# tlepoint/fhe.rs

Measured on NVIDIA B200. Metric: bfv_ct_mul_relin_per_sec_n32768_14x62bit, higher is better.
Workload: dtype u64

## Files before the change

### bench_micro/mac_bench.cu

```cuda
#include <cstdio>
#include <cuda_runtime.h>
typedef unsigned long long u64;
typedef unsigned int u32;

template <int V>
struct Acc {
  u32 e0, e1, e2, e3, e4, o1, o2, o3;
  u64 lo, mid, hi;
  __device__ __forceinline__ void clear() { e0 = e1 = e2 = e3 = e4 = o1 = o2 = o3 = 0; lo = mid = hi = 0; }
  __device__ __forceinline__ void mac(u64 a, u64 b) {
    if (V == 0) {
      asm volatile("{\n\t.reg .u32 a0,a1,b0,b1;\n\tmov.b64 {a0,a1}, %3;\n\tmov.b64 {b0,b1}, %4;\n\t"
          "mad.wide.u32 %0, a0, b0, %0;\n\tmad.wide.u32 %1, a0, b1, %1;\n\tmad.wide.u32 %1, a1, b0, %1;\n\tmad.wide.u32 %2, a1, b1, %2;\n\t}"
          : "+l"(lo), "+l"(mid), "+l"(hi) : "l"(a), "l"(b));
    } else if (V == 1) {
      asm volatile("{\n\t.reg .u32 a0, a1, b0, b1;\n\tmov.b64 {a0, a1}, %8;\n\tmov.b64 {b0, b1}, %9;\n\t"
          "mad.lo.cc.u32 %0, a0, b0, %0;\n\tmadc.hi.cc.u32 %1, a0, b0, %1;\n\tmadc.lo.cc.u32 %2, a1, b1, %2;\n\t"
          "madc.hi.cc.u32 %3, a1, b1, %3;\n\taddc.u32 %4, %4, 0;\n\t"
          "mad.lo.cc.u32 %5, a0, b1, %5;\n\tmadc.hi.cc.u32 %6, a0, b1, %6;\n\taddc.u32 %7, %7, 0;\n\t"
          "mad.lo.cc.u32 %5, a1, b0, %5;\n\tmadc.hi.cc.u32 %6, a1, b0, %6;\n\taddc.u32 %7, %7, 0;\n\t}"
          : "+r"(e0), "+r"(e1), "+r"(e2), "+r"(e3), "+r"(e4), "+r"(o1), "+r"(o2), "+r"(o3) : "l"(a), "l"(b));
    } else {
      u64 pl, ph;
      asm volatile("{\n\t.reg .u32 a0, a1, b0, b1, p0, p1, m0, m1, q0, q1, t1, t2, t3;\n\t.reg .u64 P, M, Q;\n\t"
          "mov.b64 {a0, a1}, %2;\n\tmov.b64 {b0, b1}, %3;\n\tmul.wide.u32 P, a0, b0;\n\tmul.wide.u32 M, a0, b1;\n\t"
          "mad.wide.u32 M, a1, b0, M;\n\tmul.wide.u32 Q, a1, b1;\n\tmov.b64 {p0, p1}, P;\n\tmov.b64 {m0, m1}, M;\n\t"
          "mov.b64 {q0, q1}, Q;\n\tadd.cc.u32 t1, p1, m0;\n\taddc.cc.u32 t2, q0, m1;\n\taddc.u32 t3, q1, 0;\n\t"
          "mov.b64 %0, {p0, t1};\n\tmov.b64 %1, {t2, t3};\n\t}" : "=l"(pl), "=l"(ph) : "l"(a), "l"(b));
      asm volatile("add.cc.u64 %0, %0, %3;\n\taddc.cc.u64 %1, %1, %4;\n\taddc.u64 %2, %2, 0;" : "+l"(lo), "+l"(mid), "+l"(hi) : "l"(pl), "l"(ph));
    }
  }
  __device__ __forceinline__ u64 fin() const { return lo ^ mid ^ hi ^ e0 ^ e1 ^ e2 ^ e3 ^ e4 ^ o1 ^ o2 ^ o3; }
};

template <int V, int NACC>
__global__ void k(u64* out, u64 seed, int iters) {
  Acc<V> acc[NACC];
  u64 w[8];
#pragma unroll
  for (int i = 0; i < NACC; i++) acc[i].clear();
#pragma unroll
  for (int i = 0; i < 8; i++) w[i] = (seed * (threadIdx.x + 17 + i)) & 0x3fffffffffffffffull;
  u64 r = seed ^ threadIdx.x;
  for (int it = 0; it < iters; it++) {
#pragma unroll
    for (int u = 0; u < 8 / NACC * 1; u++) {
#pragma unroll
      for (int a = 0; a < NACC; a++) acc[a].mac(r, w[(u * NACC + a) & 7]);
      r = (r + 0x9e3779b97f4a7c15ull) & 0x3fffffffffffffffull;
    }
  }
  u64 x = 0;
#pragma unroll
  for (int i = 0; i < NACC; i++) x ^= acc[i].fin();
  out[blockIdx.x * blockDim.x + threadIdx.x] = x;
}
template <int V, int NACC>
void run(int warps_per_smsp) {
  u64* out;
  int threads = 128, blocks = 148 * warps_per_smsp, iters = 2000;
  cudaMalloc(&out, sizeof(u64) * blocks * threads);
  cudaEvent_t e0, e1;
  cudaEventCreate(&e0); cudaEventCreate(&e1);
  k<V, NACC><<<blocks, threads>>>(out, 12345, 10);
  cudaDeviceSynchronize();
  cudaEventRecord(e0);
  k<V, NACC><<<blocks, threads>>>(out, 12345, iters);
  cudaEventRecord(e1);
  cudaEventSynchronize(e1);
  float ms; cudaEventElapsedTime(&ms, e0, e1);
  int dev_clk; cudaDeviceGetAttribute(&dev_clk, cudaDevAttrClockRate, 0);
  double macs_per_warp = 8.0 * iters;
  double clk = ms * 1e-3 * (dev_clk * 1e3) / (macs_per_warp * warps_per_smsp);
  printf("V%d NACC=%d warps/SMSP=%2d : %7.3f ms -> %5.1f clk per MAC per warp (at %d MHz nominal)\n", V, NACC, warps_per_smsp, ms, clk, dev_clk / 1000);
  cudaFree(out);
}
int main() {
  for (int w : {1, 2, 4, 6, 12}) {
    run<0, 4>(w); run<1, 4>(w); run<2, 4>(w);
  }
  run<1, 1>(6); run<1, 2>(6); run<1, 8>(6); run<2, 2>(6); run<2, 1>(6);
  return 0;
}
```

### fhe_rs_b200/csrc/kernels.cu

```cuda
#include <algorithm>
#include <cstdint>
#include <cstdlib>
#include <cstring>
#include <map>
#include <mutex>
#include <vector>

#include "engine.hpp"
#include "ntt_tma.cuh"

namespace fhe_b200 {

typedef unsigned __int128 u128;

namespace {

struct EwArgs {
  u64* a;
  const u64* b;
  size_t n_words;
  u32 logn, limbs_per_poly;
  const LimbDev* limbs;
  unsigned short ids[kMaxPos];
};

template <int OP>
__global__ void ew_kernel(EwArgs A) {
  size_t i = ((size_t)blockIdx.x * blockDim.x + threadIdx.x) * 2;
  if (i >= A.n_words) return;
  const u64 p = A.limbs[A.ids[(i >> A.logn) % A.limbs_per_poly]].p;
  ulonglong2 x = *reinterpret_cast<ulonglong2*>(A.a + i);
  if (OP == EW_NEG) {
    x.x = csub(p - x.x, p);
    x.y = csub(p - x.y, p);
  } else {
    ulonglong2 y = *reinterpret_cast<const ulonglong2*>(A.b + i);
    if (OP == EW_ADD) {
      x.x = csub(x.x + y.x, p);
      x.y = csub(x.y + y.y, p);
    } else {
      x.x = csub(x.x + p - y.x, p);
      x.y = csub(x.y + p - y.y, p);
    }
  }
  *reinterpret_cast<ulonglong2*>(A.a + i) = x;
}

struct MulPlainArgs {
  u64* a;
  const u64* pt;
  u32 cts, parts, n_pt, logn, limbs_per_poly;
  u32 op;
  const LimbDev* limbs;
  unsigned short ids[kMaxPos];
};
__global__ void mul_plain_kernel(MulPlainArgs A) {
  size_t idx = (size_t)blockIdx.x * blockDim.x + threadIdx.x;
  const size_t total = ((size_t)A.cts * A.parts * A.limbs_per_poly) << A.logn;
  if (idx >= total) return;
  const u32 c = idx & ((1u << A.logn) - 1);
  const size_t row = idx >> A.logn;
  const u32 limb = row % A.limbs_per_poly;
  const u32 ct = (u32)(row / ((size_t)A.limbs_per_poly * A.parts));
  const LimbDev& M = A.limbs[A.ids[limb]];
  const u64 w = A.pt[((((size_t)(ct % A.n_pt)) * A.limbs_per_poly + limb) << A.logn) + c];
  if (A.op == 0) {
// ... 120 lines not shown
  A.out[idx] = acc.reduce(M);
}

struct ScaleArgs {
  ScalerDev S;
  const LimbDev* limbs;
  const u64* in;
  u64 *out0, *out1;
  u32 polys, out_rows_per_poly, start, n_out, split3, logn;
};

struct U256 {
  u64 w0, w1, w2, w3;
};
__device__ __forceinline__ U256 u256_from_acc(const u32 (&a)[7]) {
  U256 r;
  r.w0 = ((u64)a[1] << 32) | a[0];
  r.w1 = ((u64)a[3] << 32) | a[2];
  r.w2 = ((u64)a[5] << 32) | a[4];
  r.w3 = a[6];
  return r;
}
__device__ __forceinline__ U256 u256_add(U256 a, U256 b) {
  U256 r;
  asm("add.cc.u64 %0, %4, %8;\n\t"
      "addc.cc.u64 %1, %5, %9;\n\t"
      "addc.cc.u64 %2, %6, %10;\n\t"
      "addc.u64 %3, %7, %11;"
      : "=l"(r.w0), "=l"(r.w1), "=l"(r.w2), "=l"(r.w3)
      : "l"(a.w0), "l"(a.w1), "l"(a.w2), "l"(a.w3), "l"(b.w0), "l"(b.w1), "l"(b.w2), "l"(b.w3));
  return r;
}
__device__ __forceinline__ U256 u256_sub(U256 a, U256 b) {
  U256 r;
  asm("sub.cc.u64 %0, %4, %8;\n\t"
      "subc.cc.u64 %1, %5, %9;\n\t"
      "subc.cc.u64 %2, %6, %10;\n\t"
      "subc.u64 %3, %7, %11;"
      : "=l"(r.w0), "=l"(r.w1), "=l"(r.w2), "=l"(r.w3)
      : "l"(a.w0), "l"(a.w1), "l"(a.w2), "l"(a.w3), "l"(b.w0), "l"(b.w1), "l"(b.w2), "l"(b.w3));
  return r;
}
__device__ __forceinline__ U256 u256_mul_128(u128 v, u64 tlo, u64 thi) {
  u32 a[7] = {0, 0, 0, 0, 0, 0, 0}, b[7] = {0, 0, 0, 0, 0, 0, 0};
  mac_theta(a, (u64)v, tlo, thi);
  mac_theta(b, (u64)(v >> 64), tlo, thi);
  U256 lo = u256_from_acc(a), hi = u256_from_acc(b);
  U256 hs = {0, hi.w0, hi.w1, hi.w2};
  return u256_add(lo, hs);
}

constexpr int kScaleTC = 128;

template <int G, int UNR = 2>
__device__ __forceinline__ void scale_mac_group(Acc192 (&acc)[4], const u64* r_col, const ulonglong2* om, u32 nf,
                                                u32 om_stride) {
#pragma unroll UNR
  for (u32 i = 0; i < nf; i++) {
    const u64 r = r_col[i * kScaleTC];
    const ulonglong2 o0 = om[(size_t)i * om_stride];
    acc[0].mac(r, o0.x);
    if (G > 1) acc[1].mac(r, o0.y);
    if (G > 2) {
      const ulonglong2 o1 = om[(size_t)i * om_stride + 1];
      acc[2].mac(r, o1.x);
      if (G > 3) acc[3].mac(r, o1.y);
    }
  }
}

__global__ void __launch_bounds__(kScaleTC) scale_kernel(ScaleArgs A) {
  extern __shared__ __align__(16) u64 smem[];
  const ScalerDev& S = A.S;
  const u32 nf = S.n_from, n_out = A.n_out;
  const u32 n_out4 = (n_out + 3) & ~3u;
  constexpr u32 TC = kScaleTC;
  u64* s_r = smem;
  u64* s_omega = s_r + (size_t)nf * TC;
  u64* s_gamma = s_omega + (size_t)nf * n_out4;
  u64* s_tgl = s_gamma + n_out4;
  u64* s_tgh = s_tgl + nf;
  u64* s_tol = s_tgh + nf;
  u64* s_toh = s_tol + nf;
  u32* s_ord = reinterpret_cast<u32*>(s_toh + nf);

  const u32 N = 1u << A.logn;
  const u32 per_poly = N / TC;
  const u32 poly = blockIdx.x / per_poly;
  const u32 c0 = (blockIdx.x % per_poly) * TC;
  const u64* src = A.in + (((size_t)poly * nf) << A.logn) + c0;
  const u32 cc = threadIdx.x;

  {
    const u32 dst0 = (u32)__cvta_generic_to_shared(s_r + cc);
    for (u32 i = 0; i < nf; i++)
      asm volatile("cp.async.ca.shared.global [%0], [%1], 8;" ::"r"(dst0 + i * TC * 8u),
                   "l"(src + ((size_t)i << A.logn) + cc)
                   : "memory");
    asm volatile("cp.async.commit_group;" ::: "memory");
  }
  for (u32 idx = cc; idx < nf * n_out4; idx += TC) {
    const u32 ii = idx / n_out4, jj = idx - ii * n_out4;
    s_omega[idx] = jj < n_out ? S.omega[(size_t)(A.start + jj) * nf + ii] : 0;
  }
  for (u32 i = cc; i < n_out4; i += TC) s_gamma[i] = i < n_out ? S.gamma[A.start + i] : 0;
  for (u32 i = cc; i < nf; i += TC) {
    s_tgl[i] = S.tgar_lo[i];
    s_tgh[i] = S.tgar_hi[i];
    s_tol[i] = S.to_lo[i];
    s_toh[i] = S.to_hi[i];
    s_ord[i] = i < S.n_terms ? S.to_order[i] : 0;
  }
  asm volatile("cp.async.wait_all;" ::: "memory");
  __syncthreads();

  u128 v;
  {
    AccTheta at;
    at.clear();
#pragma unroll 2
    for (u32 i = 0; i < nf; i++) at.mac(s_r[i * TC + cc], s_tgl[i], s_tgh[i]);
    u32 acc[7];
    at.words(acc);
    U256 sg = u256_from_acc(acc);
    const u32 bs = S.shift - 1 - 64;
    u64 lo = (sg.w1 >> bs) | (sg.w2 << (64 - bs));
    u64 hi = (sg.w2 >> bs) | (sg.w3 << (64 - bs));
    u128 x = ((u128)hi << 64) | lo;
    v = (x >> 1) + (x & 1);
  }
  bool w_sign = false;
  u128 w = 0;
  if (!S.is_one) {
    U256 s_pos = {0, 0, 0, 0}, s_neg = {0, 0, 0, 0};
#pragma unroll 1
    for (u32 sg = 0; sg < 2; sg++) {
      AccTheta at;
      at.clear();
      const u32 k0 = sg ? S.n_pos : 0, k1 = sg ? S.n_terms : S.n_pos;
#pragma unroll 2
      for (u32 k = k0; k < k1; k++) {
        const u32 i = s_ord[k];
        at.mac(s_r[i * TC + cc], s_tol[i], s_toh[i]);
      }
      u32 wds[7];
      at.words(wds);
      if (sg == 0) s_pos = u256_from_acc(wds);
      else s_neg = u256_from_acc(wds);
    }
    U256 so = u256_sub(s_pos, s_neg);
    U256 vt = u256_mul_128(v, S.tg_lo, S.tg_hi);
    so = S.tg_sign ? u256_add(so, vt) : u256_sub(so, vt);
    w_sign = (so.w3 != 0) || (so.w2 >> 63);
    if (w_sign) {
      u64 n1 = ~so.w1, n2 = ~so.w2, n3 = ~so.w3;
      u128 y = ((u128)((n2 >> 62) | (n3 << 2)) << 64) | ((n1 >> 62) | (n2 << 2));
      w = (y + 1) >> 1;
    } else {
      u128 y = ((u128)((so.w2 >> 62) | (so.w3 << 2)) << 64) | ((so.w1 >> 62) | (so.w2 << 2));
      w = (y >> 1) + (y & 1);
    }
  }

  for (u32 j0 = 0; j0 < n_out; j0 += 4) {
    Acc192 acc[4];
#pragma unroll
    for (int k = 0; k < 4; k++) acc[k].clear();
    const ulonglong2* om = reinterpret_cast<const ulonglong2*>(s_omega + j0);
    switch (min(4u, n_out - j0)) {
      case 4: scale_mac_group<4>(acc, s_r + cc, om, nf, n_out4 / 2); break;
      case 3: scale_mac_group<3>(acc, s_r + cc, om, nf, n_out4 / 2); break;
      case 2: scale_mac_group<2>(acc, s_r + cc, om, nf, n_out4 / 2); break;
      default: scale_mac_group<1>(acc, s_r + cc, om, nf, n_out4 / 2); break;
    }
#pragma unroll
    for (int k = 0; k < 4; k++) {
      const u32 jj = j0 + k;
      if (jj >= n_out) break;
      const LimbDev& M = A.limbs[S.to_ids[A.start + jj]];
      u64 vr = reduce94_limb((u64)v, (u64)(v >> 64), M);
      acc[k].mac(vr ? M.p - vr : 0, s_gamma[jj]);
      if (!S.is_one) {
        u64 wr = reduce94_limb((u64)w, (u64)(w >> 64), M);
        acc[k].add64(w_sign ? (wr ? M.p - wr : 0) : wr);
      }
      u64 y = acc[k].reduce(M);
      u64* dst;
      if (A.split3) {
        u32 ct = poly / 3, part = poly % 3;
        dst = part < 2 ? A.out0 + ((((size_t)ct * 2 + part) * n_out + jj) << A.logn)
                       : A.out1 + (((size_t)ct * n_out + jj) << A.logn);
      } else {
        dst = A.out0 + (((size_t)poly * A.out_rows_per_poly + jj) << A.logn);
      }
      dst[c0 + cc] = y;
    }
  }
}


struct ScaleTmaArgs {
  ScalerDev S;
  const LimbDev* limbs;
  u64 *out0, *out1;
  u32 polys, out_rows_per_poly, start, n_out, split3, logn;
  u32 tiles_total;
};

template <bool IS_ONE, int UNR>
__global__ void __launch_bounds__(kScaleTC) scale_tma_kernel(const __grid_constant__ CUtensorMap tm_in, const ScaleTmaArgs A) {
  using namespace tma;
  extern __shared__ __align__(128) u64 smem[];
  const ScalerDev& S = A.S;
  const u32 nf = S.n_from, n_out = A.n_out;
  const u32 n_out4 = (n_out + 3) & ~3u;
  constexpr u32 TC = kScaleTC;
  u64* s_r = smem;
  u64* s_omega = s_r + (size_t)nf * TC;
  u64* s_gamma = s_omega + (size_t)nf * n_out4;
  u64* s_p2 = s_gamma + n_out4;
  u64* s_c = s_p2 + n_out4;
  u64* s_tgl = s_c + n_out4;
  u64* s_tgh = s_tgl + nf;
  u64* s_tol = s_tgh + nf;
  u64* s_toh = s_tol + nf;
  u32* s_ord = reinterpret_cast<u32*>(s_toh + nf);
  u64* s_bar = reinterpret_cast<u64*>(s_ord + ((nf + 1) & ~1u));
  const u32 bar = smem_u32(s_bar);
  const u32 cc = threadIdx.x;

  for (u32 idx = cc; idx < nf * n_out4; idx += TC) {
    const u32 ii = idx / n_out4, jj = idx - ii * n_out4;
    s_omega[idx] = jj < n_out ? S.omega[(size_t)(A.start + jj) * nf + ii] : 0;
  }
  for (u32 i = cc; i < n_out4; i += TC) {
    const bool live = i < n_out;
    const LimbDev& M = A.limbs[S.to_ids[A.start + (live ? i : 0)]];
    s_gamma[i] = live ? S.gamma[A.start + i] : 0;
    s_p2[i] = M.p2;
    s_c[i] = M.sol_c;
  }
  for (u32 i = cc; i < nf; i += TC) {
    s_tgl[i] = S.tgar_lo[i];
    s_tgh[i] = S.tgar_hi[i];
    const u32 src = (!IS_ONE && i < S.n_terms) ? S.to_order[i] : 0;
    s_tol[i] = IS_ONE ? 0 : S.to_lo[src];
    s_toh[i] = IS_ONE ? 0 : S.to_hi[src];
    s_ord[i] = src * TC * 8;
  }
  if (cc == 0) {
    mbar_init(bar, 1);
    asm volatile("fence.mbarrier_init.release.cluster;" ::: "memory");
  }
  __syncthreads();

  const u32 N = 1u << A.logn;
  const u32 per_poly = N / TC;
  const u32 dst_r = smem_u32(s_r);
  const u32 tile_bytes = nf * TC * 8;
  u32 tile = blockIdx.x;
  if (cc == 0 && tile < A.tiles_total) {
    mbar_expect_tx(bar, tile_bytes);
    load_2d(dst_r, &tm_in, (tile % per_poly) * TC, (tile / per_poly) * nf, bar);
  }
  const u32 my_r = dst_r + cc * 8;
  for (u32 it = 0; tile < A.tiles_total; tile += gridDim.x, it++) {
    const u32 poly = tile / per_poly;
    const u32 c0 = (tile - poly * per_poly) * TC;
    mbar_wait(bar, it & 1);

    u128 v;
    {
      AccTheta at;
      at.clear();
#pragma unroll 2
      for (u32 i = 0; i < nf; i++) at.mac(lds64(my_r + i * TC * 8), s_tgl[i], s_tgh[i]);
      u32 acc[7];
      at.words(acc);
      U256 sg = u256_from_acc(acc);
      const u32 bs = S.shift - 1 - 64;
      u64 lo = (sg.w1 >> bs) | (sg.w2 << (64 - bs));
      u64 hi = (sg.w2 >> bs) | (sg.w3 << (64 - bs));
      u128 x = ((u128)hi << 64) | lo;
      v = (x >> 1) + (x & 1);
    }
    bool w_sign = false;
    u128 w = 0;
    if (!IS_ONE) {
      U256 s_pos = {0, 0, 0, 0}, s_neg = {0, 0, 0, 0};
#pragma unroll 1
      for (u32 sg = 0; sg < 2; sg++) {
        AccTheta at;
        at.clear();
        const u32 k0 = sg ? S.n_pos : 0, k1 = sg ? S.n_terms : S.n_pos;
#pragma unroll 2
        for (u32 k = k0; k < k1; k++) at.mac(lds64(my_r + s_ord[k]), s_tol[k], s_toh[k]);
        u32 wds[7];
        at.words(wds);
        if (sg == 0) s_pos = u256_from_acc(wds);
        else s_neg = u256_from_acc(wds);
      }
      U256 so = u256_sub(s_pos, s_neg);
      U256 vt = u256_mul_128(v, S.tg_lo, S.tg_hi);
      so = S.tg_sign ? u256_add(so, vt) : u256_sub(so, vt);
      w_sign = (so.w3 != 0) || (so.w2 >> 63);
      if (w_sign) {
        u64 n1 = ~so.w1, n2 = ~so.w2, n3 = ~so.w3;
        u128 y = ((u128)((n2 >> 62) | (n3 << 2)) << 64) | ((n1 >> 62) | (n2 << 2));
        w = (y + 1) >> 1;
      } else {
        u128 y = ((u128)((so.w2 >> 62) | (so.w3 << 2)) << 64) | ((so.w1 >> 62) | (so.w2 << 2));
        w = (y >> 1) + (y & 1);
      }
    }
    const u64 mask62 = (1ull << 62) - 1;
    const u64 vl = (u64)v & mask62, wl = (u64)w & mask62;
    const u32 vh = (u32)(v >> 62), wh = (u32)(w >> 62);

    u64* dst;
    size_t dstride = (size_t)1 << A.logn;
    if (A.split3) {
      const u32 ct = poly / 3, part = poly - ct * 3;
      dst = part < 2 ? A.out0 + ((((size_t)ct * 2 + part) * n_out) << A.logn) : A.out1 + (((size_t)ct * n_out) << A.logn);
    } else {
      dst = A.out0 + (((size_t)poly * A.out_rows_per_poly) << A.logn);
    }
    dst += c0 + cc;

    for (u32 j0 = 0; j0 < n_out; j0 += 4) {
      Acc192 acc[4];
#pragma unroll
      for (int k = 0; k < 4; k++) acc[k].clear();
      const ulonglong2* om = reinterpret_cast<const ulonglong2*>(s_omega + j0);
      const u32 g = min(4u, n_out - j0);
      switch (g) {
        case 4: scale_mac_group<4, UNR>(acc, s_r + cc, om, nf, n_out4 / 2); break;
        case 3: scale_mac_group<3, UNR>(acc, s_r + cc, om, nf, n_out4 / 2); break;
        case 2: scale_mac_group<2, UNR>(acc, s_r + cc, om, nf, n_out4 / 2); break;
        default: scale_mac_group<1, UNR>(acc, s_r + cc, om, nf, n_out4 / 2); break;
      }
      if (j0 + 4 >= n_out) {
        __syncthreads();
        const u32 nxt = tile + gridDim.x;
        if (cc == 0 && nxt < A.tiles_total) {
          mbar_expect_tx(bar, tile_bytes);
          load_2d(dst_r, &tm_in, (nxt % per_poly) * TC, (nxt / per_poly) * nf, bar);
        }
      }
#pragma unroll
      for (int k = 0; k < 4; k++) {
        const u32 jj = j0 + k;
        if (jj >= n_out) break;
        const u64 p2 = s_p2[jj];
        const u32 c = (u32)s_c[jj];
        acc[k].mac(p2 - ((u64)vh * c + vl), s_gamma[jj]);
        if (!IS_ONE) {
          const u64 wr = (u64)wh * c + wl;
          acc[k].add64(w_sign ? p2 - wr : wr);
        }
        u64 lo, mid;
        u32 hi32;
        acc[k].merged(lo, mid, hi32);
        dst[(size_t)jj * dstride] = csub(fold192_solinas(lo, mid, hi32, c), p2 >> 1);
      }
    }
  }
}

__global__ void scale_small_kernel(ScaleArgs A) {
  const ScalerDev& S = A.S;
  const u32 nf = S.n_from, n_out = A.n_out;
  const u32 N = 1u << A.logn;
  const u32 idx = blockIdx.x * blockDim.x + threadIdx.x;
  if (idx >= A.polys * N) return;
  const u32 poly = idx >> A.logn, c = idx & (N - 1);
  const u64* src = A.in + (((size_t)poly * nf) << A.logn) + c;
  u32 av[7] = {0, 0, 0, 0, 0, 0, 0}, ap[7] = {0, 0, 0, 0, 0, 0, 0}, an[7] = {0, 0, 0, 0, 0, 0, 0};
  for (u32 i = 0; i < nf; i++) {
    const u64 r = src[(size_t)i << A.logn];
    mac_theta(av, r, S.tgar_lo[i], S.tgar_hi[i]);
    if (!S.is_one) {
      if (S.to_sign[i]) mac_theta(an, r, S.to_lo[i], S.to_hi[i]);
      else mac_theta(ap, r, S.to_lo[i], S.to_hi[i]);
    }
  }
  U256 sg = u256_from_acc(av);
  const u32 bs = S.shift - 1 - 64;
  u64 lo = (sg.w1 >> bs) | (sg.w2 << (64 - bs));
  u64 hi = (sg.w2 >> bs) | (sg.w3 << (64 - bs));
  u128 x = ((u128)hi << 64) | lo;
  u128 v = (x >> 1) + (x & 1);
  bool w_sign = false;
  u128 w = 0;
  if (!S.is_one) {
    U256 so = u256_sub(u256_from_acc(ap), u256_from_acc(an));
    U256 vt = u256_mul_128(v, S.tg_lo, S.tg_hi);
    so = S.tg_sign ? u256_add(so, vt) : u256_sub(so, vt);
    w_sign = (so.w3 != 0) || (so.w2 >> 63);
    if (w_sign) {
      u64 n1 = ~so.w1, n2 = ~so.w2, n3 = ~so.w3;
      u128 y = ((u128)((n2 >> 62) | (n3 << 2)) << 64) | ((n1 >> 62) | (n2 << 2));
      w = (y + 1) >> 1;
    } else {
      u128 y = ((u128)((so.w2 >> 62) | (so.w3 << 2)) << 64) | ((so.w1 >> 62) | (so.w2 << 2));
      w = (y >> 1) + (y & 1);
    }
  }
  for (u32 j = 0; j < n_out; j++) {
    const LimbDev& M = A.limbs[S.to_ids[A.start + j]];
    Acc192 acc;
    acc.clear();
    for (u32 i = 0; i < nf; i++) acc.mac(src[(size_t)i << A.logn], S.omega[(size_t)(A.start + j) * nf + i]);
    u64 vr = reduce128_limb((u64)v, (u64)(v >> 64), M);
    acc.mac(vr ? M.p - vr : 0, S.gamma[A.start + j]);
    if (!S.is_one) {
      u64 wr = reduce128_limb((u64)w, (u64)(w >> 64), M);
// ... 355 lines not shown
namespace {
typedef CUresult (*ScaleEncodeFn)(CUtensorMap*, CUtensorMapDataType, cuuint32_t, void*, const cuuint64_t*,
                                  const cuuint64_t*, const cuuint32_t*, const cuuint32_t*, CUtensorMapInterleave,
                                  CUtensorMapSwizzle, CUtensorMapL2promotion, CUtensorMapFloatOOBfill);
ScaleEncodeFn scale_encoder() {
  static ScaleEncodeFn fn = [] {
    void* p = nullptr;
    cudaDriverEntryPointQueryResult q = cudaDriverEntryPointSymbolNotFound;
    if (cudaGetDriverEntryPoint("cuTensorMapEncodeTiled", &p, cudaEnableDefault, &q) != cudaSuccess ||
        q != cudaDriverEntryPointSuccess)
      p = nullptr;
    cudaGetLastError();
    return (ScaleEncodeFn)p;
  }();
  return fn;
}
int scale_sm_count() {
  static std::mutex mu;
  static std::map<int, int> cache;
  int dev = 0;
  FHE_CUDA(cudaGetDevice(&dev));
  std::lock_guard<std::mutex> g(mu);
  auto it = cache.find(dev);
  if (it != cache.end()) return it->second;
  int n = 0;
  FHE_CUDA(cudaDeviceGetAttribute(&n, cudaDevAttrMultiProcessorCount, dev));
  return cache[dev] = n;
}
}

static bool launch_scale_tma(const ScalerDev& S, const LimbDev* limbs, const std::vector<u64>* sol_c_of_out, const u64* in,
                             u64* out0, u64* out1, u32 polys, u32 out_rows_per_poly, u32 start, u32 n_out, int split3,
                             u32 logn, cudaStream_t st) {
  (void)sol_c_of_out;
  static const bool classic = [] { const char* e = getenv("FHE_B200_SCALER"); return e && !strcmp(e, "classic"); }();
  if (classic || !scale_encoder() || logn < 7 || (reinterpret_cast<uintptr_t>(in) & 127)) return false;
  const u32 N = 1u << logn, nf = S.n_from;
  if (nf > 64 || (u64)polys * nf >= (1ull << 31)) return false;
  CUtensorMap tm;
  const cuuint64_t gdim[2] = {N, (cuuint64_t)polys * nf};
  const cuuint64_t gstride[1] = {(cuuint64_t)8 << logn};
  const cuuint32_t box[2] = {(cuuint32_t)kScaleTC, nf};
  const cuuint32_t es[2] = {1, 1};
  if (scale_encoder()(&tm, CU_TENSOR_MAP_DATA_TYPE_UINT64, 2, (void*)in, gdim, gstride, box, es,
                      CU_TENSOR_MAP_INTERLEAVE_NONE, CU_TENSOR_MAP_SWIZZLE_NONE, CU_TENSOR_MAP_L2_PROMOTION_L2_128B,
                      CU_TENSOR_MAP_FLOAT_OOB_FILL_NONE) != CUDA_SUCCESS)
    return false;
  ScaleTmaArgs A;
  A.S = S; A.limbs = limbs; A.out0 = out0; A.out1 = out1;
  A.polys = polys; A.out_rows_per_poly = out_rows_per_poly; A.start = start; A.n_out = n_out;
  A.split3 = split3; A.logn = logn;
  A.tiles_total = polys * (N / kScaleTC);
  const size_t n_out4 = (n_out + 3) & ~(size_t)3;
  const size_t smem = (nf * kScaleTC + nf * n_out4 + 3 * n_out4 + 4 * nf) * sizeof(u64) + ((nf + 1) & ~(size_t)1) * 4 + 16;
  auto resident = [&](const void* k) {
    ensure_dynamic_smem(k, smem);
    int per_sm = 0;
    FHE_CUDA(cudaOccupancyMaxActiveBlocksPerMultiprocessor(&per_sm, k, kScaleTC, smem));
    return (u32)std::min<u64>(A.tiles_total, (u64)scale_sm_count() * std::max(per_sm, 1));
  };
  static const int unr = [] { const char* e = getenv("FHE_B200_SCALE_UNROLL"); return e ? atoi(e) : 2; }();
  if (unr == 4) {
    if (S.is_one) scale_tma_kernel<true, 4><<<resident((const void*)scale_tma_kernel<true, 4>), kScaleTC, smem, st>>>(tm, A);
    else scale_tma_kernel<false, 4><<<resident((const void*)scale_tma_kernel<false, 4>), kScaleTC, smem, st>>>(tm, A);
  } else {
    if (S.is_one) scale_tma_kernel<true, 2><<<resident((const void*)scale_tma_kernel<true, 2>), kScaleTC, smem, st>>>(tm, A);
    else scale_tma_kernel<false, 2><<<resident((const void*)scale_tma_kernel<false, 2>), kScaleTC, smem, st>>>(tm, A);
  }
  g_launches++;
  return true;
}

void launch_scale(const ScalerDev& S, const LimbDev* limbs, const u64* in, u64* out0, u64* out1, u32 polys,
                  u32 out_rows_per_poly, u32 start, u32 n_out, int split3, u32 logn, cudaStream_t st) {
  if (!polys || !n_out) return;
  if (S.all_solinas && launch_scale_tma(S, limbs, nullptr, in, out0, out1, polys, out_rows_per_poly, start, n_out, split3,
                                        logn, st))
    return;
  ScaleArgs A;
  A.S = S; A.limbs = limbs; A.in = in; A.out0 = out0; A.out1 = out1;
  A.polys = polys; A.out_rows_per_poly = out_rows_per_poly; A.start = start; A.n_out = n_out;
  A.split3 = split3; A.logn = logn;
  const u32 N = 1u << logn;
  if (N < (u32)kScaleTC) {
    const u32 total = polys * N;
    scale_small_kernel<<<(total + 63) / 64, 64, 0, st>>>(A);
    g_launches++;
    return;
  }
  const size_t n_out4 = (n_out + 3) & ~(size_t)3, nf = S.n_from;
  const size_t smem = (nf * kScaleTC + nf * n_out4 + n_out4 + 5 * nf) * sizeof(u64);
  ensure_dynamic_smem((const void*)scale_kernel, smem);
  scale_kernel<<<polys * (N / kScaleTC), kScaleTC, smem, st>>>(A);
  g_launches++;
}

void launch_ksmac(const u64* inter, const u64* k0, const u64* k1, const u64* base0, const u64* base1, u64* out0,
                  u64* out1, u32 cts, u32 n_dig, u32 Lk, u32 out_ct_rows, const RowIds& ids, const LimbDev* limbs,
                  u32 logn, cudaStream_t st, bool adjacent) {
  size_t total = ((size_t)cts * Lk) << logn;
  if (!total) return;
  static const bool classic = [] { const char* e = getenv("FHE_B200_KSMAC"); return e && !strcmp(e, "classic"); }();
  static const int stages = [] { const char* e = getenv("FHE_B200_KS_STAGES"); int v = e ? atoi(e) : 2; return v < 2 ? 2 : v > 4 ? 4 : v; }();
  const size_t smem_tma = ((size_t)(2 + stages) * n_dig * kKsTC + stages + 1) * sizeof(u64);
  if (adjacent && !classic && scale_encoder() && logn >= 7 && n_dig <= 256 && smem_tma <= 200 * 1024 &&
      !((reinterpret_cast<uintptr_t>(inter) | reinterpret_cast<uintptr_t>(k0) | reinterpret_cast<uintptr_t>(k1)) & 127) &&
      (u64)cts * Lk * n_dig < (1ull << 31)) {
    auto map = [&](const u64* base, u64 rows, CUtensorMap* m) {
      const cuuint64_t gdim[2] = {(cuuint64_t)1 << logn, rows};
      const cuuint64_t gstride[1] = {(cuuint64_t)8 << logn};
      const cuuint32_t box[2] = {(cuuint32_t)kKsTC, n_dig};
      const cuuint32_t es[2] = {1, 1};
      return scale_encoder()(m, CU_TENSOR_MAP_DATA_TYPE_UINT64, 2, (void*)base, gdim, gstride, box, es,
                             CU_TENSOR_MAP_INTERLEAVE_NONE, CU_TENSOR_MAP_SWIZZLE_NONE,
                             CU_TENSOR_MAP_L2_PROMOTION_L2_128B, CU_TENSOR_MAP_FLOAT_OOB_FILL_NONE) == CUDA_SUCCESS;
    };
    CUtensorMap mt, m0, m1;
    if (map(inter, (u64)cts * Lk * n_dig, &mt) && map(k0, (u64)Lk * n_dig, &m0) && map(k1, (u64)Lk * n_dig, &m1)) {
      KsTmaArgs T;
      T.base0 = base0; T.base1 = base1; T.out0 = out0; T.out1 = out1;
      T.cts = cts; T.n_dig = n_dig; T.Lk = Lk; T.out_ct_rows = out_ct_rows; T.logn = logn;
      T.items_total = Lk * ((1u << logn) / kKsTC) * cts;
      T.limbs = limbs;
      copy_ids(T.ids, ids);
      auto go = [&](auto kern) {
        ensure_dynamic_smem((const void*)kern, smem_tma);
        int per_sm = 0;
        FHE_CUDA(cudaOccupancyMaxActiveBlocksPerMultiprocessor(&per_sm, (const void*)kern, kKsTC, smem_tma));
        const u32 grid = (u32)std::min<u64>(T.items_total, (u64)scale_sm_count() * std::max(per_sm, 1));
        kern<<<grid, kKsTC, smem_tma, st>>>(mt, m0, m1, T);
      };
      if (stages == 2) go(ksmac_tma_kernel<2>);
      else if (stages == 3) go(ksmac_tma_kernel<3>);
      else go(ksmac_tma_kernel<4>);
      g_launches++;
      return;
    }
  }
  KsMacArgs A;
  A.adjacent = adjacent ? 1 : 0;
  A.inter = inter; A.k0 = k0; A.k1 = k1; A.base0 = base0; A.base1 = base1; A.out0 = out0; A.out1 = out1;
  A.cts = cts; A.n_dig = n_dig; A.Lk = Lk; A.out_ct_rows = out_ct_rows; A.logn = logn;
  A.limbs = limbs;
  copy_ids(A.ids, ids);
// ... 55 lines not shown
```

### fhe_rs_b200/csrc/zq.cuh

```cuda
#pragma once
#include <cstdint>
#include <cuda_runtime.h>

namespace fhe_b200 {

typedef unsigned long long u64;
typedef unsigned int u32;

struct LimbDev {
  u64 p;
  u64 p2;
  u64 bhi;
  u64 blo;
  u64 ninv;
  u64 ninv_s;
  u64 zn;
  u64 zn_s;
  u64 c128;
  u64 sol_c;
  u64 sol_ntt;
  const ulonglong2* om;
  const ulonglong2* zi;
};

__device__ __forceinline__ u64 csub(u64 x, u64 p) { return x >= p ? x - p : x; }

__device__ __forceinline__ u64 mul_shoup_lazy(u64 a, u64 w, u64 ws, u64 p) {
  const u64 q = __umul64hi(a, ws);
  const u64 np = 0 - p;
  u64 r;
  asm("{\n\t"
      ".reg .u32 a0, a1, w0, w1, q0, q1, n0, n1, lo, hi;\n\t"
      ".reg .u64 W;\n\t"
      "mov.b64 {a0, a1}, %1;\n\t"
      "mov.b64 {w0, w1}, %2;\n\t"
      "mov.b64 {q0, q1}, %3;\n\t"
      "mov.b64 {n0, n1}, %4;\n\t"
      "mul.wide.u32 W, q0, n0;\n\t"
      "mad.wide.u32 W, a0, w0, W;\n\t"
      "mov.b64 {lo, hi}, W;\n\t"
      "mad.lo.u32 hi, q0, n1, hi;\n\t"
      "mad.lo.u32 hi, q1, n0, hi;\n\t"
      "mad.lo.u32 hi, a0, w1, hi;\n\t"
      "mad.lo.u32 hi, a1, w0, hi;\n\t"
      "mov.b64 %0, {lo, hi};\n\t"
      "}"
      : "=l"(r)
      : "l"(a), "l"(w), "l"(q), "l"(np));
  return r;
}
__device__ __forceinline__ u64 mul_shoup(u64 a, u64 w, u64 ws, u64 p) {
  return csub(mul_shoup_lazy(a, w, ws, p), p);
}

__device__ __forceinline__ u64 mul_solinas_lazy(u64 y, u64 w0, u64 w1, u32 c) {
  u64 r;
  asm("{\n\t"
      ".reg .u32 y0, y1, a0, a1, b0, b1, p0, pc, q0, qc, s0, h0, h1, hh, tt, sl, r0, r1;\n\t"
      ".reg .u64 P, Q, PH, QH, PC, QC, S, R;\n\t"
      "mov.b64 {y0, y1}, %1;\n\t"
// ... 123 lines not shown
__device__ __forceinline__ u64 barrett64(u64 a, u64 p, u64 bhi, u64 blo) {
  u64 t0 = __umul64hi(a, blo);
  u64 a_lo = a * bhi, a_hi = __umul64hi(a, bhi);
  u64 s = a_lo + t0;
  u64 q = a_hi + (s < a_lo);
  return csub(a - q * p, p);
}
__device__ __forceinline__ u64 mulmod(u64 a, u64 b, u64 p, u64 bhi, u64 blo) {
  return barrett128(a * b, __umul64hi(a, b), p, bhi, blo);
}

__device__ __forceinline__ void mul128_62(u64 a, u64 b, u64& lo, u64& hi) {
  asm("{\n\t"
      ".reg .u32 a0, a1, b0, b1, p0, p1, m0, m1, q0, q1, t1, t2, t3;\n\t"
      ".reg .u64 P, M, Q;\n\t"
      "mov.b64 {a0, a1}, %2;\n\t"
      "mov.b64 {b0, b1}, %3;\n\t"
      "mul.wide.u32 P, a0, b0;\n\t"
      "mul.wide.u32 M, a0, b1;\n\t"
      "mad.wide.u32 M, a1, b0, M;\n\t"
      "mul.wide.u32 Q, a1, b1;\n\t"
      "mov.b64 {p0, p1}, P;\n\t"
      "mov.b64 {m0, m1}, M;\n\t"
      "mov.b64 {q0, q1}, Q;\n\t"
      "add.cc.u32 t1, p1, m0;\n\t"
      "addc.cc.u32 t2, q0, m1;\n\t"
      "addc.u32 t3, q1, 0;\n\t"
      "mov.b64 %0, {p0, t1};\n\t"
      "mov.b64 %1, {t2, t3};\n\t"
      "}"
      : "=l"(lo), "=l"(hi)
      : "l"(a), "l"(b));
}

__device__ __forceinline__ void fold_step_solinas(u64& lo, u64& hi, u64 top, u32 c) {
  const u64 mask = (1ull << 62) - 1;
  const u64 x = (lo >> 62) | (hi << 2);
  const u64 t0 = (u64)c * (u32)x + (lo & mask);
  const u64 t1 = (u64)c * (u32)(x >> 32) + (t0 >> 32);
  lo = (t1 << 32) | (u32)t0;
  hi = (t1 >> 32) + top * c;
}
__device__ __forceinline__ u64 fold94_solinas(u64 lo, u64 hi, u32 c) {
  const u32 x = (u32)((lo >> 62) | (hi << 2));
  return (u64)c * x + (lo & ((1ull << 62) - 1));
}
__device__ __forceinline__ u64 fold192_solinas(u64 lo, u64 mid, u64 hi, u32 c) {
  u64 top = (mid >> 62) | (hi << 2);
  fold_step_solinas(lo, mid, top, c);
  fold_step_solinas(lo, mid, 0, c);
  return fold94_solinas(lo, mid, c);
}

struct Acc192 {
  u32 e0, e1, e2, e3, e4, o1, o2, o3;
  __device__ __forceinline__ void clear() { e0 = e1 = e2 = e3 = e4 = o1 = o2 = o3 = 0; }
  __device__ __forceinline__ void mac(u64 a, u64 b) {
    asm("{\n\t"
        ".reg .u32 a0, a1, b0, b1;\n\t"
        "mov.b64 {a0, a1}, %8;\n\t"
        "mov.b64 {b0, b1}, %9;\n\t"
        "mad.lo.cc.u32 %0, a0, b0, %0;\n\t"
        "madc.hi.cc.u32 %1, a0, b0, %1;\n\t"
        "madc.lo.cc.u32 %2, a1, b1, %2;\n\t"
        "madc.hi.cc.u32 %3, a1, b1, %3;\n\t"
        "addc.u32 %4, %4, 0;\n\t"
        "mad.lo.cc.u32 %5, a0, b1, %5;\n\t"
        "madc.hi.cc.u32 %6, a0, b1, %6;\n\t"
        "addc.u32 %7, %7, 0;\n\t"
        "mad.lo.cc.u32 %5, a1, b0, %5;\n\t"
        "madc.hi.cc.u32 %6, a1, b0, %6;\n\t"
        "addc.u32 %7, %7, 0;\n\t"
        "}"
        : "+r"(e0), "+r"(e1), "+r"(e2), "+r"(e3), "+r"(e4), "+r"(o1), "+r"(o2), "+r"(o3)
        : "l"(a), "l"(b));
  }
  __device__ __forceinline__ void add64(u64 v) {
    asm("{\n\t"
        ".reg .u32 v0, v1;\n\t"
        "mov.b64 {v0, v1}, %5;\n\t"
        "add.cc.u32 %0, %0, v0;\n\t"
        "addc.cc.u32 %1, %1, v1;\n\t"
        "addc.cc.u32 %2, %2, 0;\n\t"
        "addc.cc.u32 %3, %3, 0;\n\t"
        "addc.u32 %4, %4, 0;\n\t"
        "}"
        : "+r"(e0), "+r"(e1), "+r"(e2), "+r"(e3), "+r"(e4)
        : "l"(v));
  }
  __device__ __forceinline__ void merged(u64& lo, u64& mid, u32& hi) const {
    u32 w1, w2, w3;
    asm("add.cc.u32 %0, %4, %8;\n\t"
        "addc.cc.u32 %1, %5, %9;\n\t"
        "addc.cc.u32 %2, %6, %10;\n\t"
        "addc.u32 %3, %7, 0;"
        : "=r"(w1), "=r"(w2), "=r"(w3), "=r"(hi)
        : "r"(e1), "r"(e2), "r"(e3), "r"(e4), "r"(o1), "r"(o2), "r"(o3));
    lo = ((u64)w1 << 32) | e0;
    mid = ((u64)w3 << 32) | w2;
  }
  __device__ __forceinline__ u64 reduce_lazy(const LimbDev& m) const {
    u64 lo, mid;
    u32 hi32;
    merged(lo, mid, hi32);
    const u64 hi = hi32;
    if (m.sol_c) return fold192_solinas(lo, mid, hi, (u32)m.sol_c);
    u64 r1 = barrett128_lazy(lo, mid, m.p, m.bhi, m.blo);
    u64 hl = hi * m.c128, hh = __umul64hi(hi, m.c128);
    u64 r2 = barrett128_lazy(hl, hh, m.p, m.bhi, m.blo);
    return csub(r1 + r2, m.p2);
  }
  __device__ __forceinline__ u64 reduce(const LimbDev& m) const {
    u64 lo, mid;
    u32 hi32;
    merged(lo, mid, hi32);
    const u64 hi = hi32;
    if (m.sol_c) return csub(fold192_solinas(lo, mid, hi, (u32)m.sol_c), m.p);
    u64 r1 = barrett128_lazy(lo, mid, m.p, m.bhi, m.blo);
    u64 hl = hi * m.c128, hh = __umul64hi(hi, m.c128);
    u64 r2 = barrett128_lazy(hl, hh, m.p, m.bhi, m.blo);
    return csub(csub(r1 + r2, m.p2), m.p);
  }
};

__device__ __forceinline__ u64 reduce128_limb(u64 lo, u64 hi, const LimbDev& m) {
  if (m.sol_c) return csub(fold192_solinas(lo, hi, 0, (u32)m.sol_c), m.p);
  return barrett128(lo, hi, m.p, m.bhi, m.blo);
}
__device__ __forceinline__ u64 reduce94_limb(u64 lo, u64 hi, const LimbDev& m) {
  if (m.sol_c) return csub(fold94_solinas(lo, hi, (u32)m.sol_c), m.p);
  return barrett128(lo, hi, m.p, m.bhi, m.blo);
}

__device__ __forceinline__ void mac_theta(u32 (&a)[7], u64 r, u64 tlo, u64 thi) {
  asm("{\n\t"
      ".reg .u32 r0, r1, t0, t1, t2, t3, u0, u1, u2, u3, u4, c;\n\t"
      ".reg .u64 P, C;\n\t"
      "mov.b64 {r0, r1}, %7;\n\t"
      "mov.b64 {t0, t1}, %8;\n\t"
      "mov.b64 {t2, t3}, %9;\n\t"
      "mul.wide.u32 P, r0, t0;\n\t"
      "mov.b64 {u0, c}, P;\n\t"
      "cvt.u64.u32 C, c;\n\t"
      "mad.wide.u32 P, r0, t1, C;\n\t"
      "mov.b64 {u1, c}, P;\n\t"
      "cvt.u64.u32 C, c;\n\t"
      "mad.wide.u32 P, r0, t2, C;\n\t"
      "mov.b64 {u2, c}, P;\n\t"
      "cvt.u64.u32 C, c;\n\t"
      "mad.wide.u32 P, r0, t3, C;\n\t"
      "mov.b64 {u3, u4}, P;\n\t"
      "add.cc.u32 %0, %0, u0;\n\t"
      "addc.cc.u32 %1, %1, u1;\n\t"
      "addc.cc.u32 %2, %2, u2;\n\t"
      "addc.cc.u32 %3, %3, u3;\n\t"
      "addc.cc.u32 %4, %4, u4;\n\t"
      "addc.cc.u32 %5, %5, 0;\n\t"
      "addc.u32 %6, %6, 0;\n\t"
      "mul.wide.u32 P, r1, t0;\n\t"
      "mov.b64 {u0, c}, P;\n\t"
      "cvt.u64.u32 C, c;\n\t"
      "mad.wide.u32 P, r1, t1, C;\n\t"
      "mov.b64 {u1, c}, P;\n\t"
      "cvt.u64.u32 C, c;\n\t"
      "mad.wide.u32 P, r1, t2, C;\n\t"
      "mov.b64 {u2, c}, P;\n\t"
      "cvt.u64.u32 C, c;\n\t"
      "mad.wide.u32 P, r1, t3, C;\n\t"
      "mov.b64 {u3, u4}, P;\n\t"
      "add.cc.u32 %1, %1, u0;\n\t"
      "addc.cc.u32 %2, %2, u1;\n\t"
      "addc.cc.u32 %3, %3, u2;\n\t"
      "addc.cc.u32 %4, %4, u3;\n\t"
      "addc.cc.u32 %5, %5, u4;\n\t"
// ... 81 lines not shown
```

Measured before the change: 4548.

## Use Karatsuba 31-bit split accumulator for RNS scaling MACs

```diff
diff --git a/bench_micro/mac_bench.cu b/bench_micro/mac_bench.cu
--- a/bench_micro/mac_bench.cu
+++ b/bench_micro/mac_bench.cu
@@ -55,6 +55,52 @@
   for (int i = 0; i < NACC; i++) x ^= acc[i].fin();
   out[blockIdx.x * blockDim.x + threadIdx.x] = x;
 }
+struct Acc3 {
+  u64 c00, c11, css;
+  u32 t00, t11, tss;
+  __device__ __forceinline__ void clear() { c00 = c11 = css = 0; t00 = t11 = tss = 0; }
+  __device__ __forceinline__ void mac(u32 r0, u32 r1, u32 rs, u32 w0, u32 w1, u32 ws) {
+    asm volatile("{\n\t.reg .u32 l, h;\n\t"
+        "mov.b64 {l, h}, %0;\n\tmad.lo.cc.u32 l, %6, %9, l;\n\tmadc.hi.cc.u32 h, %6, %9, h;\n\taddc.u32 %3, %3, 0;\n\tmov.b64 %0, {l, h};\n\t"
+        "mov.b64 {l, h}, %1;\n\tmad.lo.cc.u32 l, %7, %10, l;\n\tmadc.hi.cc.u32 h, %7, %10, h;\n\taddc.u32 %4, %4, 0;\n\tmov.b64 %1, {l, h};\n\t"
+        "mov.b64 {l, h}, %2;\n\tmad.lo.cc.u32 l, %8, %11, l;\n\tmadc.hi.cc.u32 h, %8, %11, h;\n\taddc.u32 %5, %5, 0;\n\tmov.b64 %2, {l, h};\n\t}"
+        : "+l"(c00), "+l"(c11), "+l"(css), "+r"(t00), "+r"(t11), "+r"(tss)
+        : "r"(r0), "r"(r1), "r"(rs), "r"(w0), "r"(w1), "r"(ws));
+  }
+  __device__ __forceinline__ u64 fin() const { return c00 ^ c11 ^ css ^ t00 ^ t11 ^ tss; }
+};
+template <int NACC>
+__global__ void k3(u64* out, u64 seed, int iters) {
+  Acc3 acc[NACC];
+  u32 w0[8], w1[8], ws[8];
+#pragma unroll
+  for (int i = 0; i < NACC; i++) acc[i].clear();
+#pragma unroll
+  for (int i = 0; i < 8; i++) {
+    const u64 w = (seed * (threadIdx.x + 17 + i)) & 0x3fffffffffffffffull;
+    w0[i] = (u32)w & 0x7fffffffu;
+    w1[i] = (u32)(w >> 31);
+    ws[i] = w0[i] + w1[i];
+  }
+  u64 r = seed ^ threadIdx.x;
+  for (int it = 0; it < iters; it++) {
+#pragma unroll
+    for (int u = 0; u < 8 / NACC * 1; u++) {
+      const u32 r0 = (u32)r & 0x7fffffffu, r1 = (u32)(r >> 31), rs = r0 + r1;
+#pragma unroll
+      for (int a = 0; a < NACC; a++) {
+        const int j = (u * NACC + a) & 7;
+        acc[a].mac(r0, r1, rs, w0[j], w1[j], ws[j]);
+      }
+      r = (r + 0x9e3779b97f4a7c15ull) & 0x3fffffffffffffffull;
+    }
+  }
+  u64 x = 0;
+#pragma unroll
+  for (int i = 0; i < NACC; i++) x ^= acc[i].fin();
+  out[blockIdx.x * blockDim.x + threadIdx.x] = x;
+}
+
 template <int V, int NACC>
 void run(int warps_per_smsp) {
   u64* out;
@@ -62,10 +108,13 @@
   cudaMalloc(&out, sizeof(u64) * blocks * threads);
   cudaEvent_t e0, e1;
   cudaEventCreate(&e0); cudaEventCreate(&e1);
-  k<V, NACC><<<blocks, threads>>>(out, 12345, 10);
+  void (*kern)(u64*, u64, int);
+  if constexpr (V == 3) kern = k3<NACC>;
+  else kern = k<V, NACC>;
+  kern<<<blocks, threads>>>(out, 12345, 10);
   cudaDeviceSynchronize();
   cudaEventRecord(e0);
-  k<V, NACC><<<blocks, threads>>>(out, 12345, iters);
+  kern<<<blocks, threads>>>(out, 12345, iters);
   cudaEventRecord(e1);
   cudaEventSynchronize(e1);
   float ms; cudaEventElapsedTime(&ms, e0, e1);
@@ -77,7 +126,7 @@
 }
 int main() {
   for (int w : {1, 2, 4, 6, 12}) {
-    run<0, 4>(w); run<1, 4>(w); run<2, 4>(w);
+    run<0, 4>(w); run<1, 4>(w); run<2, 4>(w); run<3, 4>(w);
   }
   run<1, 1>(6); run<1, 2>(6); run<1, 8>(6); run<2, 2>(6); run<2, 1>(6);
   return 0;
diff --git a/fhe_rs_b200/csrc/kernels.cu b/fhe_rs_b200/csrc/kernels.cu
--- a/fhe_rs_b200/csrc/kernels.cu
+++ b/fhe_rs_b200/csrc/kernels.cu
@@ -10,8 +10,6 @@
 #include "ntt_tma.cuh"
 
 namespace fhe_b200 {
-
-typedef unsigned __int128 u128;
 
 namespace {
 
@@ -238,20 +236,31 @@
 
 constexpr int kScaleTC = 128;
 
+__device__ __forceinline__ void stage_omega_split(u32* s_om, const ScalerDev& S, u32 start, u32 n_out, u32 n_out4,
+                                                  u32 nf) {
+  for (u32 idx = threadIdx.x; idx < nf * n_out4; idx += blockDim.x) {
+    const u32 ii = idx / n_out4, jj = idx - ii * n_out4;
+    u32 w0, w1, ws;
+    AccSplit31::split(jj < n_out ? S.omega[(size_t)(start + jj) * nf + ii] : 0, w0, w1, ws);
+    u32* d = s_om + (size_t)ii * 3 * n_out4 + (jj >> 2) * 12 + (jj & 3);
+    d[0] = w0;
+    d[4] = w1;
+    d[8] = ws;
+  }
+}
+
 template <int G, int UNR = 2>
-__device__ __forceinline__ void scale_mac_group(Acc192 (&acc)[4], const u64* r_col, const ulonglong2* om, u32 nf,
+__device__ __forceinline__ void scale_mac_group(AccSplit31 (&acc)[4], const u64* r_col, const uint4* om, u32 nf,
                                                 u32 om_stride) {
 #pragma unroll UNR
-  for (u32 i = 0; i < nf; i++) {
-    const u64 r = r_col[i * kScaleTC];
-    const ulonglong2 o0 = om[(size_t)i * om_stride];
-    acc[0].mac(r, o0.x);
-    if (G > 1) acc[1].mac(r, o0.y);
-    if (G > 2) {
-      const ulonglong2 o1 = om[(size_t)i * om_stride + 1];
-      acc[2].mac(r, o1.x);
-      if (G > 3) acc[3].mac(r, o1.y);
-    }
+  for (u32 i = 0; i < nf; i++, r_col += kScaleTC, om += om_stride) {
+    u32 r0, r1, rs;
+    AccSplit31::split(*r_col, r0, r1, rs);
+    const uint4 w0 = om[0], w1 = om[1], ws = om[2];
+    acc[0].mac(r0, r1, rs, w0.x, w1.x, ws.x);
+    if (G > 1) acc[1].mac(r0, r1, rs, w0.y, w1.y, ws.y);
+    if (G > 2) acc[2].mac(r0, r1, rs, w0.z, w1.z, ws.z);
+    if (G > 3) acc[3].mac(r0, r1, rs, w0.w, w1.w, ws.w);
   }
 }
 
@@ -262,8 +271,8 @@
   const u32 n_out4 = (n_out + 3) & ~3u;
   constexpr u32 TC = kScaleTC;
   u64* s_r = smem;
-  u64* s_omega = s_r + (size_t)nf * TC;
-  u64* s_gamma = s_omega + (size_t)nf * n_out4;
+  u32* s_om = reinterpret_cast<u32*>(s_r + (size_t)nf * TC);
+  u64* s_gamma = reinterpret_cast<u64*>(s_om + (size_t)nf * 3 * n_out4);
   u64* s_tgl = s_gamma + n_out4;
   u64* s_tgh = s_tgl + nf;
   u64* s_tol = s_tgh + nf;
@@ -285,10 +294,7 @@
                    : "memory");
     asm volatile("cp.async.commit_group;" ::: "memory");
   }
-  for (u32 idx = cc; idx < nf * n_out4; idx += TC) {
-    const u32 ii = idx / n_out4, jj = idx - ii * n_out4;
-    s_omega[idx] = jj < n_out ? S.omega[(size_t)(A.start + jj) * nf + ii] : 0;
-  }
+  stage_omega_split(s_om, S, A.start, n_out, n_out4, nf);
   for (u32 i = cc; i < n_out4; i += TC) s_gamma[i] = i < n_out ? S.gamma[A.start + i] : 0;
   for (u32 i = cc; i < nf; i += TC) {
     s_tgl[i] = S.tgar_lo[i];
@@ -349,15 +355,16 @@
   }
 
   for (u32 j0 = 0; j0 < n_out; j0 += 4) {
-    Acc192 acc[4];
+    AccSplit31 acc[4];
 #pragma unroll
     for (int k = 0; k < 4; k++) acc[k].clear();
-    const ulonglong2* om = reinterpret_cast<const ulonglong2*>(s_omega + j0);
+    const uint4* om = reinterpret_cast<const uint4*>(s_om) + j0 / 4 * 3;
+    const u32 om_stride = n_out4 / 4 * 3;
     switch (min(4u, n_out - j0)) {
-      case 4: scale_mac_group<4>(acc, s_r + cc, om, nf, n_out4 / 2); break;
-      case 3: scale_mac_group<3>(acc, s_r + cc, om, nf, n_out4 / 2); break;
-      case 2: scale_mac_group<2>(acc, s_r + cc, om, nf, n_out4 / 2); break;
-      default: scale_mac_group<1>(acc, s_r + cc, om, nf, n_out4 / 2); break;
+      case 4: scale_mac_group<4>(acc, s_r + cc, om, nf, om_stride); break;
+      case 3: scale_mac_group<3>(acc, s_r + cc, om, nf, om_stride); break;
+      case 2: scale_mac_group<2>(acc, s_r + cc, om, nf, om_stride); break;
+      default: scale_mac_group<1>(acc, s_r + cc, om, nf, om_stride); break;
     }
 #pragma unroll
     for (int k = 0; k < 4; k++) {
@@ -366,11 +373,15 @@
       const LimbDev& M = A.limbs[S.to_ids[A.start + jj]];
       u64 vr = reduce94_limb((u64)v, (u64)(v >> 64), M);
       acc[k].mac(vr ? M.p - vr : 0, s_gamma[jj]);
+      u64 add = 0;
       if (!S.is_one) {
         u64 wr = reduce94_limb((u64)w, (u64)(w >> 64), M);
-        acc[k].add64(w_sign ? (wr ? M.p - wr : 0) : wr);
+        add = w_sign ? (wr ? M.p - wr : 0) : wr;
       }
-      u64 y = acc[k].reduce(M);
+      u64 lo, mid;
+      u32 hi;
+      acc[k].merged(add, lo, mid, hi);
+      u64 y = reduce192_limb(lo, mid, hi, M);
       u64* dst;
       if (A.split3) {
         u32 ct = poly / 3, part = poly % 3;
@@ -402,8 +413,8 @@
   const u32 n_out4 = (n_out + 3) & ~3u;
   constexpr u32 TC = kScaleTC;
   u64* s_r = smem;
-  u64* s_omega = s_r + (size_t)nf * TC;
-  u64* s_gamma = s_omega + (size_t)nf * n_out4;
+  u32* s_om = reinterpret_cast<u32*>(s_r + (size_t)nf * TC);
+  u64* s_gamma = reinterpret_cast<u64*>(s_om + (size_t)nf * 3 * n_out4);
   u64* s_p2 = s_gamma + n_out4;
   u64* s_c = s_p2 + n_out4;
   u64* s_tgl = s_c + n_out4;
@@ -415,10 +426,7 @@
   const u32 bar = smem_u32(s_bar);
   const u32 cc = threadIdx.x;
 
-  for (u32 idx = cc; idx < nf * n_out4; idx += TC) {
-    const u32 ii = idx / n_out4, jj = idx - ii * n_out4;
-    s_omega[idx] = jj < n_out ? S.omega[(size_t)(A.start + jj) * nf + ii] : 0;
-  }
+  stage_omega_split(s_om, S, A.start, n_out, n_out4, nf);
   for (u32 i = cc; i < n_out4; i += TC) {
     const bool live = i < n_out;
     const LimbDev& M = A.limbs[S.to_ids[A.start + (live ? i : 0)]];
@@ -514,16 +522,17 @@
     dst += c0 + cc;
 
     for (u32 j0 = 0; j0 < n_out; j0 += 4) {
-      Acc192 acc[4];
+      AccSplit31 acc[4];
 #pragma unroll
       for (int k = 0; k < 4; k++) acc[k].clear();
-      const ulonglong2* om = reinterpret_cast<const ulonglong2*>(s_omega + j0);
+      const uint4* om = reinterpret_cast<const uint4*>(s_om) + j0 / 4 * 3;
+      const u32 om_stride = n_out4 / 4 * 3;
       const u32 g = min(4u, n_out - j0);
       switch (g) {
-        case 4: scale_mac_group<4, UNR>(acc, s_r + cc, om, nf, n_out4 / 2); break;
-        case 3: scale_mac_group<3, UNR>(acc, s_r + cc, om, nf, n_out4 / 2); break;
-        case 2: scale_mac_group<2, UNR>(acc, s_r + cc, om, nf, n_out4 / 2); break;
-        default: scale_mac_group<1, UNR>(acc, s_r + cc, om, nf, n_out4 / 2); break;
+        case 4: scale_mac_group<4, UNR>(acc, s_r + cc, om, nf, om_stride); break;
+        case 3: scale_mac_group<3, UNR>(acc, s_r + cc, om, nf, om_stride); break;
+        case 2: scale_mac_group<2, UNR>(acc, s_r + cc, om, nf, om_stride); break;
+        default: scale_mac_group<1, UNR>(acc, s_r + cc, om, nf, om_stride); break;
       }
       if (j0 + 4 >= n_out) {
         __syncthreads();
@@ -537,17 +546,18 @@
       for (int k = 0; k < 4; k++) {
         const u32 jj = j0 + k;
         if (jj >= n_out) break;
-        const u64 p2 = s_p2[jj];
+        const u64 p2 = s_p2[jj], q = p2 >> 1;
         const u32 c = (u32)s_c[jj];
-        acc[k].mac(p2 - ((u64)vh * c + vl), s_gamma[jj]);
+        acc[k].mac(csub(p2 - ((u64)vh * c + vl), q), s_gamma[jj]);
+        u64 add = 0;
         if (!IS_ONE) {
           const u64 wr = (u64)wh * c + wl;
-          acc[k].add64(w_sign ? p2 - wr : wr);
+          add = w_sign ? p2 - wr : wr;
         }
         u64 lo, mid;
         u32 hi32;
-        acc[k].merged(lo, mid, hi32);
-        dst[(size_t)jj * dstride] = csub(fold192_solinas(lo, mid, hi32, c), p2 >> 1);
+        acc[k].merged(add, lo, mid, hi32);
+        dst[(size_t)jj * dstride] = csub(fold192_solinas(lo, mid, hi32, c), q);
       }
     }
   }
@@ -1009,7 +1019,8 @@
   A.split3 = split3; A.logn = logn;
   A.tiles_total = polys * (N / kScaleTC);
   const size_t n_out4 = (n_out + 3) & ~(size_t)3;
-  const size_t smem = (nf * kScaleTC + nf * n_out4 + 3 * n_out4 + 4 * nf) * sizeof(u64) + ((nf + 1) & ~(size_t)1) * 4 + 16;
+  const size_t smem = (nf * kScaleTC + 3 * n_out4 + 4 * nf) * sizeof(u64) + nf * 3 * n_out4 * sizeof(u32) +
+                      ((nf + 1) & ~(size_t)1) * 4 + 16;
   auto resident = [&](const void* k) {
     ensure_dynamic_smem(k, smem);
     int per_sm = 0;
@@ -1046,7 +1057,7 @@
     return;
   }
   const size_t n_out4 = (n_out + 3) & ~(size_t)3, nf = S.n_from;
-  const size_t smem = (nf * kScaleTC + nf * n_out4 + n_out4 + 5 * nf) * sizeof(u64);
+  const size_t smem = (nf * kScaleTC + n_out4 + 5 * nf) * sizeof(u64) + nf * 3 * n_out4 * sizeof(u32);
   ensure_dynamic_smem((const void*)scale_kernel, smem);
   scale_kernel<<<polys * (N / kScaleTC), kScaleTC, smem, st>>>(A);
   g_launches++;
diff --git a/fhe_rs_b200/csrc/zq.cuh b/fhe_rs_b200/csrc/zq.cuh
--- a/fhe_rs_b200/csrc/zq.cuh
+++ b/fhe_rs_b200/csrc/zq.cuh
@@ -6,6 +6,7 @@
 
 typedef unsigned long long u64;
 typedef unsigned int u32;
+typedef unsigned __int128 u128;
 
 struct LimbDev {
   u64 p;
@@ -235,6 +236,14 @@
   return fold94_solinas(lo, mid, c);
 }
 
+__device__ __forceinline__ u64 reduce192_limb(u64 lo, u64 mid, u32 hi, const LimbDev& m) {
+  if (m.sol_c) return csub(fold192_solinas(lo, mid, hi, (u32)m.sol_c), m.p);
+  u64 r1 = barrett128_lazy(lo, mid, m.p, m.bhi, m.blo);
+  u64 hl = (u64)hi * m.c128, hh = __umul64hi((u64)hi, m.c128);
+  u64 r2 = barrett128_lazy(hl, hh, m.p, m.bhi, m.blo);
+  return csub(csub(r1 + r2, m.p2), m.p);
+}
+
 struct Acc192 {
   u32 e0, e1, e2, e3, e4, o1, o2, o3;
   __device__ __forceinline__ void clear() { e0 = e1 = e2 = e3 = e4 = o1 = o2 = o3 = 0; }
@@ -295,14 +304,59 @@
   }
   __device__ __forceinline__ u64 reduce(const LimbDev& m) const {
     u64 lo, mid;
-    u32 hi32;
-    merged(lo, mid, hi32);
-    const u64 hi = hi32;
-    if (m.sol_c) return csub(fold192_solinas(lo, mid, hi, (u32)m.sol_c), m.p);
-    u64 r1 = barrett128_lazy(lo, mid, m.p, m.bhi, m.blo);
-    u64 hl = hi * m.c128, hh = __umul64hi(hi, m.c128);
-    u64 r2 = barrett128_lazy(hl, hh, m.p, m.bhi, m.blo);
-    return csub(csub(r1 + r2, m.p2), m.p);
+    u32 hi;
+    merged(lo, mid, hi);
+    return reduce192_limb(lo, mid, hi, m);
+  }
+};
+
+struct AccSplit31 {
+  u64 c00, c11, css;
+  u32 t00, t11, tss;
+  __device__ __forceinline__ static void split(u64 x, u32& x0, u32& x1, u32& xs) {
+    x0 = (u32)x & 0x7fffffffu;
+    x1 = (u32)(x >> 31);
+    xs = x0 + x1;
+  }
+  __device__ __forceinline__ void clear() { c00 = c11 = css = 0; t00 = t11 = tss = 0; }
+  __device__ __forceinline__ void mac(u32 r0, u32 r1, u32 rs, u32 w0, u32 w1, u32 ws) {
+    asm("{\n\t"
+        ".reg .u32 l, h;\n\t"
+        "mov.b64 {l, h}, %0;\n\t"
+        "mad.lo.cc.u32 l, %6, %9, l;\n\t"
+        "madc.hi.cc.u32 h, %6, %9, h;\n\t"
+        "addc.u32 %3, %3, 0;\n\t"
+        "mov.b64 %0, {l, h};\n\t"
+        "mov.b64 {l, h}, %1;\n\t"
+        "mad.lo.cc.u32 l, %7, %10, l;\n\t"
+        "madc.hi.cc.u32 h, %7, %10, h;\n\t"
+        "addc.u32 %4, %4, 0;\n\t"
+        "mov.b64 %1, {l, h};\n\t"
+        "mov.b64 {l, h}, %2;\n\t"
+        "mad.lo.cc.u32 l, %8, %11, l;\n\t"
+        "madc.hi.cc.u32 h, %8, %11, h;\n\t"
+        "addc.u32 %5, %5, 0;\n\t"
+        "mov.b64 %2, {l, h};\n\t"
+        "}"
+        : "+l"(c00), "+l"(c11), "+l"(css), "+r"(t00), "+r"(t11), "+r"(tss)
+        : "r"(r0), "r"(r1), "r"(rs), "r"(w0), "r"(w1), "r"(ws));
+  }
+  __device__ __forceinline__ void mac(u64 r, u64 w) {
+    u32 r0, r1, rs, w0, w1, ws;
+    split(r, r0, r1, rs);
+    split(w, w0, w1, ws);
+    mac(r0, r1, rs, w0, w1, ws);
+  }
+  __device__ __forceinline__ void merged(u64 add, u64& lo, u64& mid, u32& hi) const {
+    const u128 a = ((u128)t00 << 64) | c00;
+    const u128 b = ((u128)t11 << 64) | c11;
+    const u128 s = ((u128)tss << 64) | css;
+    const u128 m = s - a - b;
+    const u128 x = a + (m << 31) + add + ((u128)(u64)b << 62);
+    const u128 y = ((u128)t11 << 62) + (u64)(x >> 64);
+    lo = (u64)x;
+    mid = (u64)y;
+    hi = (u32)(y >> 64);
   }
 };
 
```

Result: no change. 4550, median of 6 (+0.0%).
